# jinggqu/NextGen-UIA

Hardware: AMD Instinct MI355X
Metric: images/sec fwd+bwd BiomedCLIP+Mona bs=256 (higher is better)
Workload: dtype bf16

## Files before the change

nextgen-uia_amd/csrc/wgrad.hip:

```cpp
#include "uia_common.h"
#include "uia_kernels.h"

namespace {

typedef __attribute__((ext_vector_type(4))) short s16x4;
typedef __attribute__((ext_vector_type(8))) short s16x8;

__device__ __forceinline__ void glds16(const char* gsrc, char* lds_wave_base) {
    __builtin_amdgcn_global_load_lds((const __attribute__((address_space(1))) void*)gsrc,
                                     (__attribute__((address_space(3))) void*)lds_wave_base, 16, 0, 0);
}
__device__ __forceinline__ s16x4 lds_tr16(const char* p) {
    return __builtin_amdgcn_ds_read_tr16_b64_v4i16((__attribute__((address_space(3))) s16x4*)p);
}

constexpr int SLAB = 128;
#ifndef WG_CHUNK_SLABS
#define WG_CHUNK_SLABS 4
#endif
constexpr int CHUNK_SLABS = WG_CHUNK_SLABS;

#ifndef WG_MIN_WAVES
#define WG_MIN_WAVES 1
#endif
struct WgradGroups {
    const bf16_t* A[4];
    const bf16_t* B[4];
    float* dW[4];
    float* dbias[4];
    unsigned long long seed[4];
};

template <bool DROPB>
__global__ __launch_bounds__(256, DROPB ? 3 : WG_MIN_WAVES) void wgrad_bf16_kernel(int M, int I, int J, const WgradGroups gp, long lda, long ldb, float alpha,
                                                          long ldw, int i_valid, int j_valid, float drop_p, long drop_ld, int drop_col0) {
    extern __shared__ __attribute__((aligned(16))) char smem[];
    const bf16_t* __restrict__ A = gp.A[blockIdx.y];
    const bf16_t* __restrict__ B = gp.B[blockIdx.y];
    float* __restrict__ dW = gp.dW[blockIdx.y];
    float* __restrict__ dbias = gp.dbias[blockIdx.y];
    const unsigned long long drop_seed = gp.seed[blockIdx.y];
    char* As = smem;
    char* Bs = smem + SLAB * 128;
    const int tid = threadIdx.x, lane = tid & 63;
    const int wave = __builtin_amdgcn_readfirstlane(tid >> 6);
    const int tiles = (I / 64) * (J / 64);
    const int xcd = blockIdx.x & 7, slot = blockIdx.x >> 3;
    const int chunk = xcd + 8 * (slot / tiles), tile = slot % tiles;
    const int tj = tile % (J / 64), ti = tile / (J / 64);
    const int m_begin = chunk * (SLAB * CHUNK_SLABS);
    if (m_begin >= M) return;
    const int li = lane & 15, g = lane >> 4, qq = li >> 2, pp = li & 3;

    f32x4 acc[4][4];
#pragma unroll
    for (int a = 0; a < 4; ++a)
#pragma unroll
        for (int b = 0; b < 4; ++b) acc[a][b] = f32x4{0.f, 0.f, 0.f, 0.f};
    const bool want_bias = dbias != nullptr && tj == 0;
    f32x4 bacc[4] = {f32x4{0.f, 0.f, 0.f, 0.f}, f32x4{0.f, 0.f, 0.f, 0.f}, f32x4{0.f, 0.f, 0.f, 0.f}, f32x4{0.f, 0.f, 0.f, 0.f}};
    const bf16x8 ones = {(bf16_t)1.f, (bf16_t)1.f, (bf16_t)1.f, (bf16_t)1.f, (bf16_t)1.f, (bf16_t)1.f, (bf16_t)1.f, (bf16_t)1.f};

    const uint32_t drop_th = dropout_thresh16(drop_p);
    const float drop_inv = 1.0f / (1.0f - drop_p);
    const int trow = 32 * wave + 4 * g + qq;
    const int tsw = (trow >> 1) & 3;
    for (int sl = 0; sl < CHUNK_SLABS; ++sl) {
        const int m0 = m_begin + sl * SLAB;
        if (m0 >= M) break;
        __syncthreads();
        if constexpr (DROPB) {
            uint4 raw[SLAB / 32];
            uint32_t keep[SLAB / 32];
#pragma unroll
            for (int i = 0; i < SLAB / 32; ++i) {
                const int q = wave + 4 * i, r = 8 * q + (lane >> 3);
                int gm = m0 + r;
                gm = gm < M ? gm : M - 1;
                const int c = ((lane & 7) ^ (((r >> 1) & 3) << 1)) * 16;
                glds16((const char*)(A + (size_t)gm * lda + (size_t)ti * 64) + c, As + q * 1024);
                raw[i] = *(const uint4*)((const char*)(B + (size_t)gm * ldb + (size_t)tj * 64) + c);
            }
#pragma unroll
            for (int i = 0; i < SLAB / 32; ++i) {
                const int q = wave + 4 * i, r = 8 * q + (lane >> 3);
                int gm = m0 + r;
                gm = gm < M ? gm : M - 1;
                const int c = ((lane & 7) ^ (((r >> 1) & 3) << 1)) * 16;
                keep[i] = dropout_keep8(drop_seed, (uint32_t)(((size_t)gm * (size_t)drop_ld + (size_t)(drop_col0 + tj * 64 + (c >> 1))) >> 3), drop_th);
            }
#pragma unroll
            for (int i = 0; i < SLAB / 32; ++i) {
                const int q = wave + 4 * i;
                bf16x8 v = __builtin_bit_cast(bf16x8, raw[i]);
#pragma unroll
                for (int e = 0; e < 8; ++e) v[e] = (bf16_t)((keep[i] >> e) & 1u ? (float)v[e] * drop_inv : 0.f);
                *(bf16x8*)(Bs + q * 1024 + lane * 16) = v;
            }
        } else {
        for (int q = wave; q < SLAB / 8; q += 4) {
            const int r = 8 * q + (lane >> 3);
            int gm = m0 + r;
            gm = gm < M ? gm : M - 1;
            const int c = ((lane & 7) ^ (((r >> 1) & 3) << 1)) * 16;
            glds16((const char*)(A + (size_t)gm * lda + (size_t)ti * 64) + c, As + q * 1024);
            glds16((const char*)(B + (size_t)gm * ldb + (size_t)tj * 64) + c, Bs + q * 1024);
        }
        }
        asm volatile("s_waitcnt vmcnt(0)" ::: "memory");
        __syncthreads();
        const bool tail = m0 + SLAB > M;
        bf16x8 af[4], bfr[4];
#pragma unroll
        for (int t = 0; t < 4; ++t) {
            const int off = trow * 128 + ((t ^ tsw) << 5) + 8 * pp;
            s16x4 alo = lds_tr16(As + off), ahi = lds_tr16(As + off + 16 * 128);
            const s16x4 blo = lds_tr16(Bs + off), bhi = lds_tr16(Bs + off + 16 * 128);
            if (tail) {
#pragma unroll
                for (int e = 0; e < 4; ++e) {
                    if (m0 + 32 * wave + 4 * g + e >= M) alo[e] = 0;
                    if (m0 + 32 * wave + 16 + 4 * g + e >= M) ahi[e] = 0;
                }
            }
            const s16x8 av = {alo[0], alo[1], alo[2], alo[3], ahi[0], ahi[1], ahi[2], ahi[3]};
            const s16x8 bv = {blo[0], blo[1], blo[2], blo[3], bhi[0], bhi[1], bhi[2], bhi[3]};
            af[t] = __builtin_bit_cast(bf16x8, av);
            bfr[t] = __builtin_bit_cast(bf16x8, bv);
        }
#pragma unroll
        for (int a = 0; a < 4; ++a)
#pragma unroll
            for (int b = 0; b < 4; ++b) acc[a][b] = __builtin_amdgcn_mfma_f32_16x16x32_bf16(af[a], bfr[b], acc[a][b], 0, 0, 0);
        if (want_bias) {
#pragma unroll
            for (int a = 0; a < 4; ++a) bacc[a] = __builtin_amdgcn_mfma_f32_16x16x32_bf16(af[a], ones, bacc[a], 0, 0, 0);
        }
    }
    __syncthreads();
    float* red = (float*)smem;
    float* mine = red + (wave & 1) * 4096;
    if (wave < 2) {
#pragma unroll
        for (int a = 0; a < 4; ++a)
#pragma unroll
            for (int b = 0; b < 4; ++b)
#pragma unroll
                for (int r = 0; r < 4; ++r)
                    mine[(16 * a + 4 * g + r) * 64 + 16 * b + li] = acc[a][b][r];
    }
    __syncthreads();
    if (wave >= 2) {
#pragma unroll
        for (int a = 0; a < 4; ++a)
#pragma unroll
            for (int b = 0; b < 4; ++b)
#pragma unroll
                for (int r = 0; r < 4; ++r)
                    mine[(16 * a + 4 * g + r) * 64 + 16 * b + li] += acc[a][b][r];
    }
    __syncthreads();
#ifndef WG_NO_ATOMIC
    for (int e = tid; e < 4096; e += 256) {
        const float v = red[e] + red[4096 + e];
        const int i = ti * 64 + (e >> 6), j = tj * 64 + (e & 63);
        if (i < i_valid && j < j_valid) atomicAdd(dW + (size_t)i * ldw + j, v * alpha);
    }
#endif
    if (want_bias) {
        __syncthreads();
        if (li == 0) {
#pragma unroll
            for (int a = 0; a < 4; ++a)
#pragma unroll
                for (int r = 0; r < 4; ++r) red[wave * 64 + 16 * a + 4 * g + r] = bacc[a][r];
        }
        __syncthreads();
        if (tid < 64 && ti * 64 + tid < i_valid) atomicAdd(dbias + ti * 64 + tid, (red[tid] + red[64 + tid]) + (red[128 + tid] + red[192 + tid]));
    }
}

__global__ __launch_bounds__(256) void wgrad_f32_kernel(int M, int I, int J, const float* __restrict__ A, long lda,
                                                         const float* __restrict__ B, long ldb, float alpha,
                                                         float* __restrict__ dW, float* __restrict__ dbias, long ldw, int i_valid, int j_valid) {
    extern __shared__ __attribute__((aligned(16))) char smem[];
    const int tid = threadIdx.x, lane = tid & 63;
    const int wave = __builtin_amdgcn_readfirstlane(tid >> 6);
    const int tj = blockIdx.x % (J / 64), ti = blockIdx.x / (J / 64);
    const int m_begin = blockIdx.y * (SLAB * CHUNK_SLABS);
    const int m_end = min(M, m_begin + SLAB * CHUNK_SLABS);
    const int li = lane & 15, g = lane >> 4;
    f32x4 acc[4][4];
#pragma unroll
    for (int a = 0; a < 4; ++a)
#pragma unroll
        for (int b = 0; b < 4; ++b) acc[a][b] = f32x4{0.f, 0.f, 0.f, 0.f};
    float bsum = 0.f;
    for (int m = m_begin + 4 * wave; m < m_end; m += 16) {
        const int row = m + g;
        const bool ok = row < m_end;
        const int rr = ok ? row : m_end - 1;
        float av[4], bv[4];
#pragma unroll
        for (int t = 0; t < 4; ++t) {
            av[t] = ok ? A[(size_t)rr * lda + ti * 64 + 16 * t + li] : 0.f;
            bv[t] = B[(size_t)rr * ldb + tj * 64 + 16 * t + li];
            bsum += av[t];
        }
#pragma unroll
        for (int a = 0; a < 4; ++a)
#pragma unroll
            for (int b = 0; b < 4; ++b) acc[a][b] = __builtin_amdgcn_mfma_f32_16x16x4f32(av[a], bv[b], acc[a][b], 0, 0, 0);
        (void)bsum;
    }
    __syncthreads();
    float* red = (float*)smem;
#pragma unroll
    for (int a = 0; a < 4; ++a)
#pragma unroll
        for (int b = 0; b < 4; ++b)
#pragma unroll
            for (int r = 0; r < 4; ++r) red[wave * 4096 + (16 * a + 4 * g + r) * 64 + 16 * b + li] = acc[a][b][r];
    __syncthreads();
    for (int e = tid; e < 4096; e += 256) {
        const float v = red[e] + red[4096 + e] + red[8192 + e] + red[12288 + e];
        const int i = ti * 64 + (e >> 6), j = tj * 64 + (e & 63);
        if (i < i_valid && j < j_valid) atomicAdd(dW + (size_t)i * ldw + j, v * alpha);
    }
    if (dbias && tj == 0) {
        const int col = tid & 63, part = tid >> 6;
        float s = 0.f;
        for (int m = m_begin + part; m < m_end; m += 4) s += A[(size_t)m * lda + ti * 64 + col];
        __syncthreads();
        red[tid] = s;
        __syncthreads();
        if (tid < 64 && ti * 64 + tid < i_valid) atomicAdd(dbias + ti * 64 + tid, red[tid] + red[64 + tid] + red[128 + tid] + red[192 + tid]);
    }
}

}

int uia_wgrad_group_launch(hipStream_t stream, int dtype, int n, int M, int I, int J, const void* const* A, long lda, const void* const* B, long ldb, float alpha,
                            float* const* dW, float* const* dbias, long ldw, int i_valid, int j_valid, float drop_p, const uint64_t* drop_seed, long drop_ld, int drop_col0) {
    if (ldw == 0) { ldw = J; i_valid = I; j_valid = J; }
    UIA_CHECK_ARG(dtype == UIA_BF16 || dtype == UIA_F32, "uia_wgrad: bad dtype %d", dtype);
    UIA_CHECK_ARG(n >= 1 && n <= 4 && (n == 1 || dtype == UIA_BF16), "uia_wgrad_group: 1..4 problems per launch (bf16), got %d", n);
    UIA_CHECK_ARG(M > 0 && I > 0 && J > 0 && I % 64 == 0 && J % 64 == 0, "uia_wgrad: I=%d and J=%d must be multiples of 64 (M=%d)", I, J, M);
    const int esz = dtype == UIA_BF16 ? 2 : 4;
    UIA_CHECK_ARG((lda * esz) % 16 == 0 && (ldb * esz) % 16 == 0, "uia_wgrad: alignment");
    UIA_CHECK_ARG(lda >= I && ldb >= J, "uia_wgrad: leading dimension too small");
    UIA_CHECK_ARG(i_valid > 0 && i_valid <= I && j_valid > 0 && j_valid <= J && ldw >= j_valid, "uia_wgrad: valid extent %d x %d (ldw %ld) outside the padded %d x %d", i_valid, j_valid, ldw, I, J);
    WgradGroups gp = {};
    for (int g = 0; g < n; ++g) {
        UIA_CHECK_ARG(A[g] && B[g] && dW[g] && (uintptr_t)A[g] % 16 == 0 && (uintptr_t)B[g] % 16 == 0, "uia_wgrad: null or misaligned tensor (problem %d)", g);
        gp.A[g] = (const bf16_t*)A[g]; gp.B[g] = (const bf16_t*)B[g]; gp.dW[g] = dW[g]; gp.dbias[g] = dbias ? dbias[g] : nullptr; gp.seed[g] = drop_seed ? drop_seed[g] : 0;
    }
    const int chunks = (M + SLAB * CHUNK_SLABS - 1) / (SLAB * CHUNK_SLABS);
    const dim3 grid_f32((I / 64) * (J / 64), chunks);
    const dim3 grid(8 * ((chunks + 7) / 8) * (I / 64) * (J / 64), n);
    const int lds = 4 * 4096 * 4;
    const int lds_bf16 = 2 * SLAB * 128;
    static UiaDevOnce once_bf16, once_f32;
    UIA_CHECK_ARG(drop_p >= 0.f && drop_p < 1.f, "uia_wgrad: drop_p=%f outside [0, 1)", (double)drop_p);
    UIA_CHECK_ARG(drop_p == 0.f || (dtype == UIA_BF16 && drop_ld >= drop_col0 + J && drop_col0 >= 0 && drop_col0 % 8 == 0 && drop_ld % 8 == 0 && (size_t)M * (size_t)drop_ld / 8 <= 0xFFFFFFFFull),
                  "uia_wgrad: dropout on the B operand needs bf16, a window of J columns at a multiple of 8 inside rows of drop_ld (a multiple of 8) elements, M*drop_ld <= 2^35");
    UIA_ENSURE_LDS_ATTR(once_bf16, wgrad_bf16_kernel<false>, lds_bf16);
    UIA_ENSURE_LDS_ATTR(once_f32, wgrad_f32_kernel, lds);
    if (dtype == UIA_BF16)
        if (drop_p > 0.f) {
            static UiaDevOnce once_drop;
            UIA_ENSURE_LDS_ATTR(once_drop, wgrad_bf16_kernel<true>, lds_bf16);
            hipLaunchKernelGGL(wgrad_bf16_kernel<true>, grid, dim3(256), lds_bf16, stream, M, I, J, gp, lda, ldb, alpha, ldw, i_valid, j_valid, drop_p, drop_ld, drop_col0);
        } else
        hipLaunchKernelGGL(wgrad_bf16_kernel<false>, grid, dim3(256), lds_bf16, stream, M, I, J, gp, lda, ldb, alpha, ldw, i_valid, j_valid, 0.f, 0l, 0);
    else
        hipLaunchKernelGGL(wgrad_f32_kernel, grid_f32, dim3(256), lds, stream, M, I, J, (const float*)A[0], lda, (const float*)B[0], ldb, alpha, dW[0], dbias ? dbias[0] : nullptr, ldw, i_valid, j_valid);
    UIA_CHECK_LAUNCH();
    return 0;
}

int uia_wgrad_launch(hipStream_t stream, int dtype, int M, int I, int J, const void* A, long lda, const void* B, long ldb, float alpha,
                     float* dW, float* dbias, long ldw, int i_valid, int j_valid, float drop_p, uint64_t drop_seed, long drop_ld, int drop_col0) {
    UIA_CHECK_ARG(A && B && dW, "uia_wgrad: null tensor");
    return uia_wgrad_group_launch(stream, dtype, 1, M, I, J, &A, lda, &B, ldb, alpha, &dW, &dbias, ldw, i_valid, j_valid, drop_p, &drop_seed, drop_ld, drop_col0);
}
```

Before: 6420.

## Add multi-stage LDS ring wgrad kernel for narrow bf16 weight gradients

Adds a new bf16 weight-gradient kernel used when a single ungrouped problem has I or J equal to 64 and no dropout. Each wave runs a private multi-stage LDS ring fed by direct global-to-LDS loads, with explicit vmcnt waits, so loads stay several slabs ahead of the MFMA work. The M dimension is split into row chunks sized to fill roughly a fixed number of workgroups, and work items are mapped per XCD. The intent is better latency hiding and occupancy for the skinny Mona adapter projections. The cost is much more LDS per workgroup, hand-written inline asm waits, and more atomics when there are many chunks.

```diff
diff --git a/nextgen-uia_amd/csrc/wgrad.hip b/nextgen-uia_amd/csrc/wgrad.hip
--- a/nextgen-uia_amd/csrc/wgrad.hip
+++ b/nextgen-uia_amd/csrc/wgrad.hip
@@ -180,6 +180,175 @@
     }
 }
 
+#ifndef WG_RING_STAGES
+#define WG_RING_STAGES 4
+#endif
+#ifndef WG_RING_WGS
+#define WG_RING_WGS 256
+#endif
+#ifndef WG_RING_MIN_SLABS
+#define WG_RING_MIN_SLABS 4
+#endif
+constexpr int RING = WG_RING_STAGES;
+constexpr int RING_WGS = WG_RING_WGS;
+constexpr int RING_MIN_SLABS = WG_RING_MIN_SLABS;
+constexpr int RING_STAGE = 2 * 32 * 128;
+static_assert(RING >= 2 && RING <= 5, "the vmcnt ladder below covers two to five stages");
+
+__device__ __forceinline__ void ring_wait(int ahead) {
+    if (ahead >= 4) asm volatile("s_waitcnt vmcnt(32)" ::: "memory");
+    else if (ahead == 3) asm volatile("s_waitcnt vmcnt(24)" ::: "memory");
+    else if (ahead == 2) asm volatile("s_waitcnt vmcnt(16)" ::: "memory");
+    else if (ahead == 1) asm volatile("s_waitcnt vmcnt(8)" ::: "memory");
+    else asm volatile("s_waitcnt vmcnt(0)" ::: "memory");
+}
+
+__device__ __forceinline__ s16x4 ring_tr16(const char* p, int byte_offset) {
+    s16x4 r;
+    const uint32_t a = (uint32_t)(uintptr_t)(const __attribute__((address_space(3))) char*)p;
+    asm volatile("ds_read_b64_tr_b16 %0, %1 offset:%2" : "=v"(r) : "v"(a), "n"(byte_offset));
+    return r;
+}
+__device__ __forceinline__ void ring_reads_done(s16x4 (&a)[4], s16x4 (&b)[4], s16x4 (&c)[4], s16x4 (&d)[4]) {
+    asm volatile("s_waitcnt lgkmcnt(0)" : "+v"(a[0]), "+v"(a[1]), "+v"(a[2]), "+v"(a[3]), "+v"(b[0]), "+v"(b[1]), "+v"(b[2]), "+v"(b[3]) : : "memory");
+    asm volatile("" : "+v"(c[0]), "+v"(c[1]), "+v"(c[2]), "+v"(c[3]), "+v"(d[0]), "+v"(d[1]), "+v"(d[2]), "+v"(d[3]) : : "memory");
+    __builtin_amdgcn_sched_barrier(0);
+}
+
+__global__ __launch_bounds__(256) void wgrad_bf16_ring_kernel(int M, int I, int J, const bf16_t* __restrict__ A, const bf16_t* __restrict__ B, float* __restrict__ dW,
+                                                              float* __restrict__ dbias, long lda, long ldb, float alpha, long ldw, int i_valid, int j_valid,
+                                                              int slabs, int chunks) {
+    extern __shared__ __attribute__((aligned(16))) char smem[];
+    const int tid = threadIdx.x, lane = tid & 63;
+    const int wave = __builtin_amdgcn_readfirstlane(tid >> 6);
+    const int tiles = (I / 64) * (J / 64);
+    const long items = (long)chunks * tiles;
+    const int xcd = blockIdx.x & 7;
+    const int item = (int)(xcd * items / 8) + (int)(blockIdx.x >> 3);
+    if (item >= (int)((xcd + 1) * items / 8)) return;
+    const int chunk = item / tiles, tile = item % tiles;
+    const int tj = tile % (J / 64), ti = tile / (J / 64);
+    const int s_begin = (int)((long)chunk * slabs / chunks);
+    const int n = (int)((long)(chunk + 1) * slabs / chunks) - s_begin;
+    const int li = lane & 15, g = lane >> 4, qq = li >> 2, pp = li & 3;
+
+    f32x4 acc[4][4];
+#pragma unroll
+    for (int a = 0; a < 4; ++a)
+#pragma unroll
+        for (int b = 0; b < 4; ++b) acc[a][b] = f32x4{0.f, 0.f, 0.f, 0.f};
+    const bool want_bias = dbias != nullptr && tj == 0;
+    f32x4 bacc[4] = {f32x4{0.f, 0.f, 0.f, 0.f}, f32x4{0.f, 0.f, 0.f, 0.f}, f32x4{0.f, 0.f, 0.f, 0.f}, f32x4{0.f, 0.f, 0.f, 0.f}};
+    const bf16x8 ones = {(bf16_t)1.f, (bf16_t)1.f, (bf16_t)1.f, (bf16_t)1.f, (bf16_t)1.f, (bf16_t)1.f, (bf16_t)1.f, (bf16_t)1.f};
+
+    char* ring = smem + wave * (RING * RING_STAGE);
+    const int srow = lane >> 3;
+    const int scol = ((lane & 7) ^ (((srow >> 1) & 3) << 1)) * 16;
+    const char* Ag = (const char*)(A + (size_t)ti * 64) + scol;
+    const char* Bg = (const char*)(B + (size_t)tj * 64) + scol;
+    auto stage = [&](int it, int buf) {
+        char* dst = ring + buf * RING_STAGE;
+        const int m0 = (s_begin + it) * SLAB + 32 * wave + srow;
+#pragma unroll
+        for (int i = 0; i < 4; ++i) {
+            int gm = m0 + 8 * i;
+            gm = gm < M ? gm : M - 1;
+            glds16(Ag + (size_t)gm * (size_t)lda * 2, dst + i * 1024);
+            glds16(Bg + (size_t)gm * (size_t)ldb * 2, dst + 4096 + i * 1024);
+        }
+    };
+    const int lrow = 4 * g + qq;
+    const int tsw = (lrow >> 1) & 3;
+
+    const int pre = n < RING - 1 ? n : RING - 1;
+    for (int it = 0; it < pre; ++it) stage(it, it);
+    int rbuf = 0, wbuf = pre % RING;
+    for (int it = 0; it < n; ++it) {
+        int ahead = n - 1 - it;
+        if (ahead >= RING - 1) {
+            stage(it + RING - 1, wbuf);
+            wbuf = wbuf + 1 == RING ? 0 : wbuf + 1;
+            ahead = RING - 1;
+        }
+        ring_wait(ahead);
+        const char* As = ring + rbuf * RING_STAGE;
+        rbuf = rbuf + 1 == RING ? 0 : rbuf + 1;
+        const int m0 = (s_begin + it) * SLAB + 32 * wave;
+        const bool tail = m0 + 32 > M;
+        bf16x8 af[4], bfr[4];
+        s16x4 alo4[4], ahi4[4], blo4[4], bhi4[4];
+#pragma unroll
+        for (int t = 0; t < 4; ++t) {
+            const int off = lrow * 128 + ((t ^ tsw) << 5) + 8 * pp;
+            alo4[t] = ring_tr16(As + off, 0), ahi4[t] = ring_tr16(As + off, 16 * 128);
+            blo4[t] = ring_tr16(As + off, 4096), bhi4[t] = ring_tr16(As + off, 4096 + 16 * 128);
+        }
+        ring_reads_done(alo4, ahi4, blo4, bhi4);
+#pragma unroll
+        for (int t = 0; t < 4; ++t) {
+            s16x4 alo = alo4[t], ahi = ahi4[t];
+            const s16x4 blo = blo4[t], bhi = bhi4[t];
+            if (tail) {
+#pragma unroll
+                for (int e = 0; e < 4; ++e) {
+                    if (m0 + 4 * g + e >= M) alo[e] = 0;
+                    if (m0 + 16 + 4 * g + e >= M) ahi[e] = 0;
+                }
+            }
+            const s16x8 av = {alo[0], alo[1], alo[2], alo[3], ahi[0], ahi[1], ahi[2], ahi[3]};
+            const s16x8 bv = {blo[0], blo[1], blo[2], blo[3], bhi[0], bhi[1], bhi[2], bhi[3]};
+            af[t] = __builtin_bit_cast(bf16x8, av);
+            bfr[t] = __builtin_bit_cast(bf16x8, bv);
+        }
+#pragma unroll
+        for (int a = 0; a < 4; ++a)
+#pragma unroll
+            for (int b = 0; b < 4; ++b) acc[a][b] = __builtin_amdgcn_mfma_f32_16x16x32_bf16(af[a], bfr[b], acc[a][b], 0, 0, 0);
+        if (want_bias) {
+#pragma unroll
+            for (int a = 0; a < 4; ++a) bacc[a] = __builtin_amdgcn_mfma_f32_16x16x32_bf16(af[a], ones, bacc[a], 0, 0, 0);
+        }
+    }
+    asm volatile("s_waitcnt lgkmcnt(0)" ::: "memory");
+    __syncthreads();
+    float* red = (float*)smem;
+    float* mine = red + (wave & 1) * 4096;
+    if (wave < 2) {
+#pragma unroll
+        for (int a = 0; a < 4; ++a)
+#pragma unroll
+            for (int b = 0; b < 4; ++b)
+#pragma unroll
+                for (int r = 0; r < 4; ++r) mine[(16 * a + 4 * g + r) * 64 + 16 * b + li] = acc[a][b][r];
+    }
+    __syncthreads();
+    if (wave >= 2) {
+#pragma unroll
+        for (int a = 0; a < 4; ++a)
+#pragma unroll
+            for (int b = 0; b < 4; ++b)
+#pragma unroll
+                for (int r = 0; r < 4; ++r) mine[(16 * a + 4 * g + r) * 64 + 16 * b + li] += acc[a][b][r];
+    }
+    __syncthreads();
+    for (int e = tid; e < 4096; e += 256) {
+        const float v = red[e] + red[4096 + e];
+        const int i = ti * 64 + (e >> 6), j = tj * 64 + (e & 63);
+        if (i < i_valid && j < j_valid) atomicAdd(dW + (size_t)i * ldw + j, v * alpha);
+    }
+    if (want_bias) {
+        __syncthreads();
+        if (li == 0) {
+#pragma unroll
+            for (int a = 0; a < 4; ++a)
+#pragma unroll
+                for (int r = 0; r < 4; ++r) red[wave * 64 + 16 * a + 4 * g + r] = bacc[a][r];
+        }
+        __syncthreads();
+        if (tid < 64 && ti * 64 + tid < i_valid) atomicAdd(dbias + ti * 64 + tid, (red[tid] + red[64 + tid]) + (red[128 + tid] + red[192 + tid]));
+    }
+}
+
 __global__ __launch_bounds__(256) void wgrad_f32_kernel(int M, int I, int J, const float* __restrict__ A, long lda,
                                                          const float* __restrict__ B, long ldb, float alpha,
                                                          float* __restrict__ dW, float* __restrict__ dbias, long ldw, int i_valid, int j_valid) {
@@ -266,7 +435,17 @@
                   "uia_wgrad: dropout on the B operand needs bf16, a window of J columns at a multiple of 8 inside rows of drop_ld (a multiple of 8) elements, M*drop_ld <= 2^35");
     UIA_ENSURE_LDS_ATTR(once_bf16, wgrad_bf16_kernel<false>, lds_bf16);
     UIA_ENSURE_LDS_ATTR(once_f32, wgrad_f32_kernel, lds);
-    if (dtype == UIA_BF16)
+    if (dtype == UIA_BF16 && n == 1 && drop_p == 0.f && (I == 64 || J == 64)) {
+        const int slabs = (M + SLAB - 1) / SLAB, tiles = (I / 64) * (J / 64);
+        const int by_cus = RING_WGS / tiles, by_rows = slabs / RING_MIN_SLABS;
+        const int row_chunks = std::max(1, std::min(by_cus, by_rows));
+        const int lds_ring = 4 * RING * RING_STAGE;
+        static UiaDevOnce once_ring;
+        UIA_ENSURE_LDS_ATTR(once_ring, wgrad_bf16_ring_kernel, lds_ring);
+        const long items = (long)row_chunks * tiles;
+        hipLaunchKernelGGL(wgrad_bf16_ring_kernel, dim3((unsigned)(8 * ((items + 7) / 8))), dim3(256), lds_ring, stream, M, I, J, gp.A[0], gp.B[0], gp.dW[0], gp.dbias[0],
+                           lda, ldb, alpha, ldw, i_valid, j_valid, slabs, row_chunks);
+    } else if (dtype == UIA_BF16)
         if (drop_p > 0.f) {
             static UiaDevOnce once_drop;
             UIA_ENSURE_LDS_ATTR(once_drop, wgrad_bf16_kernel<true>, lds_bf16);
```

New measurement: 6437, median of 6. No clear change (+0.3%).
